# jrached/trajectory_generator_ros2

Hardware: AMD Instinct MI355X
Metric: min-snap trajectories/sec (10-seg, order-7, 3-axis) at batch=65k; 1/2/4/8 GPU (higher is better)
Workload: dtype f64

## Files before the change

include/tgms.h:

```cpp
#ifndef TGMS_H
#define TGMS_H

#include <stdint.h>

#ifdef __cplusplus
extern "C" {
#endif

#define TGMS_ABI_VERSION 2
#define TGMS_MAX_SEGMENTS 16
#define TGMS_DENSE_MAX_SEGMENTS 10
#define TGMS_GOAL_STRIDE 14

typedef enum tgms_status {
    TGMS_OK = 0,
    TGMS_ERR_INVALID_ARG = 1,
    TGMS_ERR_SINGULAR = 2,
    TGMS_ERR_NONFINITE = 3,
    TGMS_ERR_NO_DEVICE = 4,
    TGMS_ERR_DEVICE = 5,
    TGMS_ERR_UNSUPPORTED = 6,
    TGMS_ERR_SKIPPED = 7
} tgms_status;

// ... 6 lines not shown
typedef enum tgms_yaw_mode {
    TGMS_YAW_CONSTANT = 0,
    TGMS_YAW_VELOCITY = 1
} tgms_yaw_mode;

typedef struct tgms_handle tgms_handle;

int tgms_abi_version(void);
const char* tgms_status_string(int status);

tgms_status tgms_create(tgms_handle** out, int device);
tgms_status tgms_create_host(tgms_handle** out);
void tgms_destroy(tgms_handle* h);
const char* tgms_last_error(const tgms_handle* h);
tgms_status tgms_set_method(tgms_handle* h, int method);

tgms_status tgms_solve_batch(tgms_handle* h, int32_t B, const int32_t* seg_offsets,
                             const double* waypoints, const double* seg_times,
                             const double* end_derivs, double* coeffs, int32_t* status);

tgms_status tgms_solve_uniform_device(tgms_handle* h, int32_t B, int32_t M,
                                      const double* d_waypoints, const double* d_seg_times,
                                      const double* d_end_derivs, double* d_coeffs,
                                      int32_t* d_status, void* stream);
tgms_status tgms_solve_batch_device(tgms_handle* h, int32_t B, const int32_t* h_seg_offsets,
                                    const int32_t* d_seg_offsets, const double* d_waypoints,
                                    const double* d_seg_times, const double* d_end_derivs,
                                    double* d_coeffs, int32_t* d_status, void* stream);

tgms_status tgms_refine_uniform_device(tgms_handle* h, int32_t B, int32_t M, const double* d_waypoints,
// ... 8 lines not shown
                                    const int32_t* d_seg_offsets, const double* d_waypoints, double* d_seg_times,
                                    const double* d_end_derivs, double k_T, double eta, int32_t iters,
                                    double* d_coeffs, double* d_cost, int32_t* d_status, void* stream);
tgms_status tgms_refine_batch(tgms_handle* h, int32_t B, const int32_t* seg_offsets, const double* waypoints,
                              double* seg_times, const double* end_derivs, double k_T, double eta, int32_t iters,
                              double* coeffs, double* cost, int32_t* status);

int64_t tgms_sample_count(double total_T, double dt);
tgms_status tgms_sample_offsets(int32_t B, const int32_t* seg_offsets, const double* seg_times,
                                double dt, int64_t* sample_offsets);
tgms_status tgms_sample_batch(tgms_handle* h, int32_t B, const int32_t* seg_offsets,
                              const double* waypoints, const double* seg_times,
                              const double* end_derivs, const double* coeffs, double dt,
                              int yaw_mode, double yaw_const, const int64_t* sample_offsets,
                              double* out);
tgms_status tgms_sample_batch_device(tgms_handle* h, int32_t B, const int32_t* d_seg_offsets,
                                     const double* d_waypoints, const double* d_seg_times,
                                     const double* d_end_derivs, const double* d_coeffs,
                                     double dt, int yaw_mode, double yaw_const,
                                     const int64_t* d_sample_offsets, double* d_out,
                                     void* stream);

#define TGMS_EXTREMA_STRIDE 10
#define TGMS_FEAS_BOX 1
#define TGMS_FEAS_SPEED 2
#define TGMS_FEAS_ACCEL 4
#define TGMS_FEAS_JERK 8
#define TGMS_FEAS_NONFINITE 16
typedef struct tgms_limits {
    double pmin[3], pmax[3], v_max, a_max, j_max;
// ... 282 lines not shown
```

trajectory_generator_ros2_amd/_lib.py:

```python
from __future__ import annotations

import ctypes
import os

from .build import LIB_TGMS

OK, ERR_INVALID_ARG, ERR_SINGULAR, ERR_NONFINITE, ERR_NO_DEVICE, ERR_DEVICE, ERR_UNSUPPORTED, ERR_SKIPPED = range(8)
METHOD_REDUCED, METHOD_DENSE_KKT, METHOD_BAND_KKT = 0, 1, 2
YAW_CONSTANT, YAW_VELOCITY = 0, 1
ABI_VERSION = 2
MAX_SEGMENTS = 16
DENSE_MAX_SEGMENTS = 10
GOAL_STRIDE = 14
EXTREMA_STRIDE = 10
FEAS_BOX, FEAS_SPEED, FEAS_ACCEL, FEAS_JERK, FEAS_NONFINITE = 1, 2, 4, 8, 16
SEP_STRIDE = 2
SEP_CLOSE, SEP_NONFINITE = 1, 16
NEAR_NONE = -1
CLR_BAD_OBSTACLE = 32
FLD_UNRESOLVED = 64
INF_BLOCKED, INF_OUTSIDE, INF_CAPPED = 1, 2, 4
SUB_DONE, SUB_FULL, SUB_BLOCKED, SUB_OUTSIDE = 1, 2, 4, 8
SUB_MAX_DEPTH = 4
THRUST_STRIDE = 6
THRUST_LOW, THRUST_HIGH, THRUST_TILT = 1, 2, 4
RATE_STRIDE = 2
RATE_HIGH = 1
DIL_CAPPED = 1
DIL_FLAG_MASK, DIL_EVALS_SHIFT = 0xFF, 8
DIL_NONE, DIL_SPEED, DIL_ACCEL, DIL_JERK, DIL_THRUST_HIGH, DIL_THRUST_LOW, DIL_TILT = range(7)
COR_STRIDE = 2
COR_MAX_FACES = 256
COR_OUTSIDE, COR_BAD_FACE = 1, 32
SPLIT_PULL, SPLIT_CHORD = 0, 1
SPLIT_DONE, SPLIT_FULL, SPLIT_AT_END = 1, 2, 4
CUT_DONE, CUT_SNAPPED, CUT_FINISHED = 1, 2, 4

EXPORTS = [
    "tgms_abi_version", "tgms_status_string", "tgms_create", "tgms_create_host", "tgms_destroy", "tgms_last_error",
    "tgms_set_method", "tgms_solve_batch", "tgms_solve_uniform_device", "tgms_solve_batch_device",
    "tgms_sample_count", "tgms_sample_offsets", "tgms_sample_batch", "tgms_sample_batch_device",
    "tgms_refine_uniform_device", "tgms_refine_batch_device", "tgms_refine_loop_device", "tgms_refine_batch",
    "tgms_create_multi", "tgms_device_count", "tgms_plan_shards", "tgms_solve_batch_multi",
    "tgms_solve_batch_multi_device", "tgms_refine_loop_multi_device", "tgms_multi_schedule",
    "tgms_extrema_batch", "tgms_extrema_batch_device", "tgms_bounds_batch", "tgms_bounds_batch_device",
    "tgms_separation_batch", "tgms_separation_batch_device",
    "tgms_neighbors_batch", "tgms_neighbors_batch_device",
    "tgms_clearance_batch", "tgms_clearance_batch_device",
    "tgms_field_clearance_batch", "tgms_field_clearance_batch_device",
    "tgms_field_occupancy_device", "tgms_corridor_inflate_batch", "tgms_corridor_inflate_batch_device",
    "tgms_corridor_subdivide_batch", "tgms_corridor_subdivide_batch_device",
    "tgms_thrust_batch", "tgms_thrust_batch_device",
    "tgms_rate_batch", "tgms_rate_batch_device",
    "tgms_dilate_batch", "tgms_dilate_batch_device",
    "tgms_corridor_batch", "tgms_corridor_batch_device",
    "tgms_corridor_split_batch", "tgms_corridor_split_batch_device",
    "tgms_cut_batch", "tgms_cut_batch_device",
]

SCHED_REFINE, SCHED_END_DERIVS, SCHED_COEFFS, SCHED_STATUS, SCHED_COST, SCHED_SELF_GATHER = 1, 2, 4, 8, 16, 32


class Piece(ctypes.Structure):
    _fields_ = [("dev", ctypes.c_int32), ("piece", ctypes.c_int32), ("lo", ctypes.c_int32), ("hi", ctypes.c_int32),
                ("s0", ctypes.c_int64), ("s1", ctypes.c_int64), ("ws_off", ctypes.c_int64 * 11)]


class Xfer(ctypes.Structure):
    _fields_ = [("dev", ctypes.c_int32), ("piece", ctypes.c_int32), ("gather", ctypes.c_int32),
                ("array", ctypes.c_int32), ("batch_elem", ctypes.c_int64), ("ws_byte", ctypes.c_int64),
                ("count", ctypes.c_int64), ("elem_bytes", ctypes.c_int32), ("group", ctypes.c_int32)]

# ... 153 lines not shown
    L.tgms_dilate_batch.restype = ctypes.c_int
    L.tgms_corridor_batch_device.argtypes = [vp, i32, vp, vp, vp, ctypes.c_int64, vp, vp, dbl, vp, vp, vp, vp, vp, vp]
    L.tgms_corridor_batch_device.restype = ctypes.c_int
    L.tgms_corridor_batch.argtypes = [vp, i32, vp, vp, vp, ctypes.c_int64, vp, vp, dbl, vp, vp, vp, vp, vp]
    L.tgms_corridor_batch.restype = ctypes.c_int
    L.tgms_corridor_split_batch_device.argtypes = [vp, i32, vp, vp, vp, vp, ctypes.c_int64, vp, vp, vp, vp, dbl,
                                                   ctypes.c_int, dbl, vp, vp, vp, vp, vp, vp, vp, vp, vp]
    L.tgms_corridor_split_batch_device.restype = ctypes.c_int
    L.tgms_corridor_split_batch.argtypes = [vp, i32, vp, vp, vp, vp, ctypes.c_int64, vp, vp, vp, vp, dbl,
                                            ctypes.c_int, dbl, vp, vp, vp, vp, vp, vp, vp, vp]
    L.tgms_corridor_split_batch.restype = ctypes.c_int
    L.tgms_cut_batch_device.argtypes = [vp, i32, vp, vp, vp, vp, vp, vp, dbl, vp, vp, vp, vp, vp, vp, vp, vp, vp, vp]
    L.tgms_cut_batch_device.restype = ctypes.c_int
    L.tgms_cut_batch.argtypes = [vp, i32, vp, vp, vp, vp, vp, vp, dbl, vp, vp, vp, vp, vp, vp, vp, vp, vp]
    L.tgms_cut_batch.restype = ctypes.c_int
    if L.tgms_abi_version() != ABI_VERSION:
        raise ImportError(f"libtgms ABI {L.tgms_abi_version()} != {ABI_VERSION}")
    _lib = L
    return L


def status_string(status: int) -> str:
    return load().tgms_status_string(int(status)).decode()
```

trajectory_generator_ros2_amd/csrc/tgms_capi.hip:

```cpp
#include <chrono>
#include <thread>
#include <initializer_list>
#include "tgms.h"
#include "tgms_internal.h"
#include "tgms_plan.h"
#include "tgms_host.h"
#include "tgms_dilate_core.h"
#include "tgms_separation_core.h"

#include <dlfcn.h>
#include <hip/hip_runtime.h>
#include <rccl/rccl.h>

#include <algorithm>
#include <cmath>
#include <cstdio>
#include <cstdlib>
#include <cstring>
#include <functional>
#include <limits>
#include <string>
#include <vector>

#ifndef TGMS_AUX_STREAMS
#define TGMS_AUX_STREAMS 4
#endif

struct tgms_multi_ctx;

struct tgms_handle {
    bool host = false;
    int device = 0;
    tgms_multi_ctx* multi = nullptr;
    int method = TGMS_METHOD_REDUCED;
    hipStream_t stream = nullptr;
    std::string last_error;
    void* d_ws = nullptr;
    size_t ws_cap = 0;
    int32_t* d_perm = nullptr;
    size_t perm_cap = 0;
    int32_t* d_perm_hist = nullptr;
    size_t perm_hist_cap = 0;
    tgms::DevPlan* d_plan = nullptr;
    int32_t* h_perm = nullptr;
    size_t h_perm_cap = 0;
    hipEvent_t perm_ev = nullptr;
    hipEvent_t scratch_ev = nullptr;
    bool scratch_pending = false;
    double* d_loop_ws = nullptr;
    size_t loop_ws_cap = 0;
    void* d_nbr_ws = nullptr;
    size_t nbr_ws_cap = 0;
    hipStream_t aux[TGMS_AUX_STREAMS] = {};
// ... 51 lines not shown
        if (e_ != hipSuccess) return hip_err(h, e_, #call); \
    } while (0)

size_t align256(size_t x) { return (x + 255) & ~size_t(255); }

tgms_status ensure_ws(tgms_handle* h, size_t bytes) {
    if (bytes <= h->ws_cap) return TGMS_OK;
    if (h->d_ws) {
        TGMS_HIP(h, hipStreamSynchronize(h->stream));
        TGMS_HIP(h, hipFree(h->d_ws));
        h->d_ws = nullptr;
        h->ws_cap = 0;
    }
    TGMS_HIP(h, hipMalloc(&h->d_ws, bytes));
    h->ws_cap = bytes;
    return TGMS_OK;
}

tgms_status enter(tgms_handle* h, const char* gpu_only = nullptr) {
    if (!h) return TGMS_ERR_INVALID_ARG;
    if (gpu_only && h->host)
        return set_err(h, TGMS_ERR_UNSUPPORTED, std::string(gpu_only) + " needs a GPU handle (tgms_create)");
    h->last_error.clear();
    return TGMS_OK;
}

struct Region {
    void* slot;
    void (*set)(void* slot, char*);
    const void* src;
    size_t bytes;
};
template <class T>
void set_slot(void* slot, char* p) {
    *static_cast<T**>(slot) = reinterpret_cast<T*>(p);
}
template <class T>
Region input(T** dev, const T* src, size_t n) {
    return {dev, set_slot<T>, src, src ? n * sizeof(T) : 0};
}
template <class T>
Region output(T** dev, size_t n) {
    return {dev, set_slot<T>, nullptr, n * sizeof(T)};
}

tgms_status stage(tgms_handle* h, std::initializer_list<Region> regions) {
    TGMS_HIP(h, hipSetDevice(h->device));
    size_t off = 0;
    for (const Region& r : regions) off = align256(off + r.bytes);
    const tgms_status s = ensure_ws(h, off);
    if (s != TGMS_OK) return s;
    char* const base = static_cast<char*>(h->d_ws);
    off = 0;
    for (const Region& r : regions) {
        char* const d = r.bytes ? base + off : nullptr;
        r.set(r.slot, d);
        if (d && r.src) TGMS_HIP(h, hipMemcpyAsync(d, r.src, r.bytes, hipMemcpyHostToDevice, h->stream));
        off = align256(off + r.bytes);
    }
    return TGMS_OK;
}

template <class T>
hipError_t fetch(tgms_handle* h, T* host, const T* dev, size_t n) {
    return hipMemcpyAsync(host, dev, n * sizeof(T), hipMemcpyDeviceToHost, h->stream);
}

struct Outputs {
    template <class T>
    struct Part {
        size_t i;
    };
    struct Slot {
        void* host;
        size_t off, bytes;
    };
    std::vector<Slot> slots;
    size_t bytes = 0;
    char* d = nullptr;
    std::vector<char> all;

    template <class T>
    Part<T> add(T* host, size_t cap, bool reserve) {
        const size_t n = reserve ? cap * sizeof(T) : 0, off = (bytes + 15) & ~size_t(15);
        if (n) bytes = off + n;
        slots.push_back({n ? host : nullptr, off, n});
        return {slots.size() - 1};
    }
    template <class T>
    Part<T> add(T* host, size_t cap) {
        return add(host, cap, host != nullptr);
    }
    template <class T>
    T* dev(Part<T> p) const {
        return slots[p.i].bytes ? reinterpret_cast<T*>(d + slots[p.i].off) : nullptr;
    }

    tgms_status copy(tgms_handle* h, void* dst, size_t off, size_t n) const {
        TGMS_HIP(h, hipMemcpyAsync(dst, d + off, n, hipMemcpyDeviceToHost, h->stream));
        TGMS_HIP(h, hipStreamSynchronize(h->stream));
        return TGMS_OK;
    }
    tgms_status fetch(tgms_handle* h) {
        all.resize(bytes);
        return copy(h, all.data(), 0, bytes);
    }
    template <class T>
    void take(Part<T> p, size_t n) const {
        if (slots[p.i].host) std::memcpy(slots[p.i].host, all.data() + slots[p.i].off, n * sizeof(T));
    }
    tgms_status download(tgms_handle* h) {
        const Slot* only = nullptr;
        int wanted = 0;
        for (const Slot& s : slots)
            if (s.host) {
                only = &s;
                ++wanted;
            }
        if (wanted == 1) return copy(h, only->host, only->off, only->bytes);
        const tgms_status st = fetch(h);
        for (const Slot& s : slots)
            if (st == TGMS_OK && s.host) std::memcpy(s.host, all.data() + s.off, s.bytes);
        return st;
    }
};
Region output(Outputs* o) { return output(&o->d, o->bytes); }

tgms_status worst_status(tgms_handle* h, const int32_t* st, int32_t B, bool message) {
    int worst = TGMS_OK;
    for (int32_t b = 0; b < B; ++b) worst = std::max(worst, (int)st[b]);
    if (worst != TGMS_OK && message) {
        for (int32_t b = 0; b < B; ++b)
            if (st[b] == worst) {
                char buf[160];
                snprintf(buf, sizeof buf, "trajectory %d: %s", b, tgms_status_string(worst));
                h->last_error = buf;
                break;
            }
    }
    return (tgms_status)worst;
}

tgms_status finish_status(tgms_handle* h, const int32_t* dSt, int32_t* status, int32_t B, bool message) {
    std::vector<int32_t> tmp;
    if (!status) {
        tmp.resize(B);
        status = tmp.data();
    }
    TGMS_HIP(h, fetch(h, status, dSt, (size_t)B));
    TGMS_HIP(h, hipStreamSynchronize(h->stream));
    return worst_status(h, status, B, message);
}

bool capturing(hipStream_t stream) {
    hipStreamCaptureStatus cs = hipStreamCaptureStatusNone;
    return hipStreamIsCapturing(stream, &cs) == hipSuccess && cs != hipStreamCaptureStatusNone;
}

tgms_status scratch_acquire(tgms_handle* h, hipStream_t stream) {
    if (h->scratch_pending && !capturing(stream)) TGMS_HIP(h, hipStreamWaitEvent(stream, h->scratch_ev, 0));
    return TGMS_OK;
}

tgms_status scratch_release(tgms_handle* h, hipStream_t stream) {
    if (capturing(stream)) return TGMS_OK;
    TGMS_HIP(h, hipEventRecord(h->scratch_ev, stream));
// ... 1048 lines not shown
        case TGMS_ERR_DEVICE: return "TGMS_ERR_DEVICE";
        case TGMS_ERR_UNSUPPORTED: return "TGMS_ERR_UNSUPPORTED";
        case TGMS_ERR_SKIPPED: return "TGMS_ERR_SKIPPED";
        default: return "TGMS_ERR_UNKNOWN";
    }
}

tgms_status tgms_create(tgms_handle** out, int device) {
    if (!out) return TGMS_ERR_INVALID_ARG;
    *out = nullptr;
    int n = 0;
    if (hipGetDeviceCount(&n) != hipSuccess || n <= 0) return TGMS_ERR_NO_DEVICE;
    if (device < 0 || device >= n) return TGMS_ERR_INVALID_ARG;
    tgms_handle* h = new tgms_handle();
    h->device = device;
    if (hipSetDevice(device) != hipSuccess ||
        hipStreamCreateWithFlags(&h->stream, hipStreamNonBlocking) != hipSuccess ||
        hipEventCreateWithFlags(&h->perm_ev, hipEventDisableTiming) != hipSuccess ||
        hipEventCreateWithFlags(&h->scratch_ev, hipEventDisableTiming) != hipSuccess) {
        delete h;
        return TGMS_ERR_DEVICE;
    }
    *out = h;
    return TGMS_OK;
}

tgms_status tgms_create_host(tgms_handle** out) {
    if (!out) return TGMS_ERR_INVALID_ARG;
    tgms_handle* h = new tgms_handle();
    h->host = true;
// ... 3 lines not shown

void tgms_destroy(tgms_handle* h) {
    if (!h) return;
    if (h->host) {
        delete h;
        return;
    }
    if (h->multi) {
        destroy_multi(h->multi);
        h->multi = nullptr;
    }
    (void)hipSetDevice(h->device);
    if (h->stream) (void)hipStreamSynchronize(h->stream);
    (void)hipDeviceSynchronize();
    if (h->d_ws) (void)hipFree(h->d_ws);
    if (h->d_perm_hist) (void)hipFree(h->d_perm_hist);
    if (h->d_band) (void)hipFree(h->d_band);
    if (h->d_band_graph) (void)hipFree(h->d_band_graph);
    for (double* p : h->band_retired) (void)hipFree(p);
    if (h->d_perm) (void)hipFree(h->d_perm);
    if (h->h_perm) (void)hipHostFree(h->h_perm);
    if (h->perm_ev) (void)hipEventDestroy(h->perm_ev);
    if (h->scratch_ev) (void)hipEventDestroy(h->scratch_ev);
    if (h->band_done) (void)hipHostFree(h->band_done);
    if (h->d_loop_ws) (void)hipFree(h->d_loop_ws);
    if (h->d_nbr_ws) (void)hipFree(h->d_nbr_ws);
    for (int j = 0; j < TGMS_AUX_STREAMS; ++j) {
        if (h->aux[j]) (void)hipStreamDestroy(h->aux[j]);
        if (h->join_ev[j]) (void)hipEventDestroy(h->join_ev[j]);
    }
    if (h->fork_ev) (void)hipEventDestroy(h->fork_ev);
    for (auto& g : h->loop_graphs) {
        if (g.done) (void)hipEventSynchronize(g.done);
        if (g.exec) (void)hipGraphExecDestroy(g.exec);
        if (g.done) (void)hipEventDestroy(g.done);
    }
    if (h->d_plan) (void)hipFree(h->d_plan);
    if (h->cap_stream) (void)hipStreamDestroy(h->cap_stream);
    if (h->stream) (void)hipStreamDestroy(h->stream);
    (void)hipGetLastError();
    delete h;
}

const char* tgms_last_error(const tgms_handle* h) { return h ? h->last_error.c_str() : ""; }

tgms_status tgms_set_method(tgms_handle* h, int method) {
    if (!h) return TGMS_ERR_INVALID_ARG;
    if (method != TGMS_METHOD_REDUCED && method != TGMS_METHOD_DENSE_KKT && method != TGMS_METHOD_BAND_KKT)
        return set_err(h, TGMS_ERR_INVALID_ARG, "unknown method");
    if (h->host && method != TGMS_METHOD_REDUCED)
        return set_err(h, TGMS_ERR_UNSUPPORTED, "the host backend solves the reduced formulation only");
    h->method = method;
    if (h->multi)
        for (tgms_handle* sub : h->multi->sub)
            if (sub) sub->method = method;
    return TGMS_OK;
}

tgms_status tgms_solve_batch(tgms_handle* h, int32_t B, const int32_t* so, const double* waypoints,
                             const double* seg_times, const double* end_derivs, double* coeffs,
// ... 8 lines not shown
    if (h->host) {
        int worst = TGMS_OK;
        for (int32_t b = 0; b < B; ++b) {
            const int64_t s0 = so[b];
            const int st = tgms::host::solve(so[b + 1] - so[b], waypoints + (s0 + b) * 3, seg_times + s0,
                                             end_derivs ? end_derivs + (int64_t)b * 18 : nullptr, coeffs + s0 * 24);
            if (status) status[b] = st;
            if (st > worst) {
                worst = st;
                h->last_error = "trajectory " + std::to_string(b) + ": " + tgms_status_string(st);
            }
        }
        return (tgms_status)worst;
    }
    const size_t S = (size_t)so[B];
    double *dW, *dT, *dED, *dC;
    int32_t *dSt, *dSo;
    s = stage(h, {input(&dW, waypoints, (S + B) * 3), input(&dT, seg_times, S), input(&dED, end_derivs, (size_t)B * 18),
                  output(&dC, S * 24), output(&dSt, (size_t)B), input(&dSo, so, (size_t)B + 1)});
    if (s != TGMS_OK) return s;
    hipStream_t st = h->stream;
    s = scratch_acquire(h, st);
    if (s != TGMS_OK) return s;
    s = plan_upload(h, B, so, &plan, st);
    if (s != TGMS_OK) return s;
    s = scratch_release(h, st, dispatch(h, plan, B, dSo, dW, dT, dED, dC, dSt, st));
    if (s != TGMS_OK) return s;
    TGMS_HIP(h, fetch(h, coeffs, dC, S * 24));
    return finish_status(h, dSt, status, B, true);
}

static bool misaligned(std::initializer_list<const void*> ps) {
    for (const void* p : ps)
        if (p && (reinterpret_cast<uintptr_t>(p) & 15u)) return true;
    return false;
}
#define TGMS_CHECK_ALIGNED(h, ...)                                                                   \
    do {                                                                                             \
        if (misaligned({__VA_ARGS__}))                                                               \
            return set_err(h, TGMS_ERR_INVALID_ARG, "fp64 device buffers must be 16-byte aligned"); \
    } while (0)

tgms_status tgms_solve_uniform_device(tgms_handle* h, int32_t B, int32_t M, const double* dW,
                                      const double* dT, const double* dED, double* dC,
// ... 82 lines not shown
}

tgms_status tgms_refine_batch(tgms_handle* h, int32_t B, const int32_t* so, const double* waypoints,
                              double* seg_times, const double* end_derivs, double k_T, double eta, int32_t iters,
                              double* coeffs, double* cost, int32_t* status) {
    if (tgms_status e = enter(h, __func__); e != TGMS_OK) return e;
    tgms_status s = check_refine_args(h, k_T, eta);
    if (s != TGMS_OK) return s;
    if (iters < 0) return set_err(h, TGMS_ERR_INVALID_ARG, "iters < 0");
    Plan plan;
    s = scan_offsets(h, B, so, TGMS_MAX_SEGMENTS, &plan.uniform_m);
    if (s != TGMS_OK) return s;
    if (B == 0) return TGMS_OK;
    if (!waypoints || !seg_times) return set_err(h, TGMS_ERR_INVALID_ARG, "NULL waypoints/seg_times");
    const size_t S = (size_t)so[B];
    double *dW, *dT[2], *dED, *dC, *dCost;
    int32_t *dSt, *dSo;
    s = stage(h, {input(&dW, waypoints, (S + B) * 3), input(&dT[0], seg_times, S), output(&dT[1], S),
                  input(&dED, end_derivs, (size_t)B * 18), output(&dC, coeffs ? S * 24 : 0), output(&dCost, (size_t)B),
                  output(&dSt, (size_t)B), input(&dSo, so, (size_t)B + 1)});
    if (s != TGMS_OK) return s;
    hipStream_t st = h->stream;
    s = scratch_acquire(h, st);
    if (s == TGMS_OK && plan.uniform_m == 0) s = ensure_perm_device(h, B);
    if (s != TGMS_OK) return s;
    const DevPlanBufs dp{h->d_perm_hist, h->d_perm, h->d_plan};
    int cur = 0;
    s = scratch_release(h, st, refine_loop(h, plan, B, (int64_t)S, dSo, dW, dT, dED, k_T, eta, iters, dC, dCost, dSt,
                                           st, &cur, &dp));
    if (s != TGMS_OK) return s;
    if (coeffs) TGMS_HIP(h, fetch(h, coeffs, dC, S * 24));
    TGMS_HIP(h, fetch(h, seg_times, dT[cur], S));
    if (cost) TGMS_HIP(h, fetch(h, cost, dCost, (size_t)B));
    return finish_status(h, dSt, status, B, false);
}

tgms_status tgms_refine_loop_device(tgms_handle* h, int32_t B, const int32_t* h_so, const int32_t* d_so,
                                    const double* dW, double* dT, const double* dED, double k_T, double eta,
                                    int32_t iters, double* dC, double* d_cost, int32_t* dSt, void* stream) {
    if (tgms_status e = enter(h, __func__); e != TGMS_OK) return e;
    tgms_status s = check_refine_args(h, k_T, eta);
    if (s != TGMS_OK) return s;
    if (iters < 0) return set_err(h, TGMS_ERR_INVALID_ARG, "iters < 0");
    int um = 0;
    s = scan_offsets(h, B, h_so, TGMS_MAX_SEGMENTS, &um);
    if (s != TGMS_OK) return s;
    if (B == 0) return TGMS_OK;
    if (!d_so || !dW || !dT) return set_err(h, TGMS_ERR_INVALID_ARG, "NULL device pointer");
    TGMS_CHECK_ALIGNED(h, dW, dT, dED, dC, d_cost);
    hipStream_t st = static_cast<hipStream_t>(stream);
    s = no_capture(h, st, "tgms_refine_loop_device (it captures and replays its own graph)");
    if (s == TGMS_OK) s = scratch_acquire(h, st);
    if (s != TGMS_OK) return s;
    return scratch_release(h, st, loop_on_device(h, B, (int64_t)h_so[B], um, d_so, dW, dT, dED, k_T, eta, iters, dC,
                                                 d_cost, dSt, st));
}

int64_t tgms_sample_count(double total_T, double dt) {
    if (!(dt > 0.0) || !(total_T >= 0.0) || !std::isfinite(total_T)) return 0;
    const double x = std::ceil(total_T / dt - 1e-9);
    int64_t n = (int64_t)x;
    if (n < 1) n = 1;
    return n + 1;
}

tgms_status tgms_sample_offsets(int32_t B, const int32_t* so, const double* T, double dt,
                                int64_t* sample_offsets) {
    if (B < 0 || !so || !sample_offsets || (B > 0 && !T) || !(dt > 0.0)) return TGMS_ERR_INVALID_ARG;
    sample_offsets[0] = 0;
    for (int32_t b = 0; b < B; ++b) {
// ... 32 lines not shown
    if (B == 0) return TGMS_OK;
    if (!waypoints || !seg_times || !coeffs || !sample_offsets || !out || !(dt > 0.0))
        return set_err(h, TGMS_ERR_INVALID_ARG, "NULL pointer or dt <= 0");
    if (yaw_mode != TGMS_YAW_CONSTANT && yaw_mode != TGMS_YAW_VELOCITY)
        return set_err(h, TGMS_ERR_INVALID_ARG, "bad yaw_mode");
    if (h->host) {
        for (int32_t b = 0; b < B; ++b) {
            const int64_t s0 = so[b];
            tgms::host::sample(so[b + 1] - so[b], coeffs + s0 * 24, seg_times + s0, waypoints + (s0 + b) * 3,
                               end_derivs ? end_derivs + (int64_t)b * 18 : nullptr, dt, yaw_mode, yaw_const,
                               sample_offsets[b + 1] - sample_offsets[b], out + sample_offsets[b] * TGMS_GOAL_STRIDE);
        }
        return TGMS_OK;
    }
    const size_t S = (size_t)so[B], nOut = (size_t)sample_offsets[B] * TGMS_GOAL_STRIDE;
    double *dW, *dT, *dED, *dC, *dOut;
    int32_t* dSo;
    int64_t* dSmp;
    s = stage(h, {input(&dW, waypoints, (S + B) * 3), input(&dT, seg_times, S), input(&dED, end_derivs, (size_t)B * 18),
                  input(&dC, coeffs, S * 24), input(&dSo, so, (size_t)B + 1),
                  input(&dSmp, sample_offsets, (size_t)B + 1), output(&dOut, nOut)});
    if (s != TGMS_OK) return s;
    TGMS_HIP(h, tgms::launch_sample(B, dSo, dW, dT, dED, dC, dt, yaw_mode, yaw_const, dSmp, dOut, h->stream));
    TGMS_HIP(h, fetch(h, out, dOut, nOut));
    TGMS_HIP(h, hipStreamSynchronize(h->stream));
    return TGMS_OK;
}


static bool resolve_limits(const tgms_limits* in, tgms_limits* out) {
    const double inf = std::numeric_limits<double>::infinity();
    if (!in) {
        *out = tgms_limits{{-inf, -inf, -inf}, {inf, inf, inf}, inf, inf, inf};
        return true;
    }
    *out = *in;
    for (int a = 0; a < 3; ++a)
        if (!(in->pmin[a] <= in->pmax[a])) return false;
    return !(std::isnan(in->v_max) || std::isnan(in->a_max) || std::isnan(in->j_max));
}

// ... 1190 lines not shown
    a.iters = iters;
    return multi_run(h, a, static_cast<hipStream_t>(stream));
}

tgms_status tgms_solve_batch_multi(tgms_handle* h, int32_t B, const int32_t* so, const double* waypoints,
                                   const double* seg_times, const double* end_derivs, double* coeffs,
                                   int32_t* status) {
    if (tgms_status e = enter(h, __func__); e != TGMS_OK) return e;
    if (!h->multi) return tgms_solve_batch(h, B, so, waypoints, seg_times, end_derivs, coeffs, status);
    Plan checked;
    tgms_status s = check_offsets(h, B, so, max_m_for(h), &checked.counts, &checked.uniform_m);
    if (s != TGMS_OK || B == 0) return s;
    if (!waypoints || !seg_times || !coeffs)
        return set_err(h, TGMS_ERR_INVALID_ARG, "NULL waypoints/seg_times/coeffs");
    const size_t S = (size_t)so[B];
    double *dW, *dT, *dED, *dC;
    int32_t *dSt, *dSo;
    s = stage(h, {input(&dW, waypoints, (S + B) * 3), input(&dT, seg_times, S), input(&dED, end_derivs, (size_t)B * 18),
                  output(&dC, S * 24), output(&dSt, (size_t)B), input(&dSo, so, (size_t)B + 1)});
    if (s != TGMS_OK) return s;
    MultiArgs a;
    a.checked = &checked;
    a.B = B;
    a.h_so = so;
    a.d_so = dSo;
    a.dW = dW;
    a.dT = dT;
    a.dED = dED;
    a.dC = dC;
    a.dSt = dSt;
    s = multi_run(h, a, h->stream);
    (void)hipSetDevice(h->device);
    if (s != TGMS_OK) return s;
    TGMS_HIP(h, fetch(h, coeffs, dC, S * 24));
    return finish_status(h, dSt, status, B, true);
}

}
```

trajectory_generator_ros2_amd/host/MinSnap.cpp:

```cpp
#include "MinSnap.hpp"

#include <algorithm>
#include <cmath>
#include <cstdlib>
#include <string>

namespace trajectory_generator {

namespace {

GoalMsg to_goal(const double* s) {
    GoalMsg g;
    g.header.frame_id = "world";
    g.p.x = s[0];
    g.p.y = s[1];
    g.p.z = s[2];
    g.v.x = s[3];
    g.v.y = s[4];
    g.v.z = s[5];
    g.a.x = s[6];
    g.a.y = s[7];
    g.a.z = s[8];
    g.j.x = s[9];
    g.j.y = s[10];
// ... 32 lines not shown
    }
    return h_;
}

bool MinSnap::solve_and_sample(const std::vector<double>& W, const std::vector<double>& T, const double* end_derivs,
                               std::vector<double>& coeffs, std::vector<double>& samples, std::string& err) {
    tgms_handle* h = handle();
    if (!h) {
        err = p_.host_backend ? "no host solver" : "no GPU solver";
        return false;
    }
    const int32_t M = (int32_t)T.size();
    const int32_t so[2] = {0, M};
    int32_t st = TGMS_OK;
    coeffs.assign((size_t)M * 24, 0.0);
    tgms_status s = tgms_solve_batch(h, 1, so, W.data(), T.data(), end_derivs, coeffs.data(), &st);
    if (s != TGMS_OK || st != TGMS_OK) {
        err = std::string("solve failed: ") + tgms_status_string(s != TGMS_OK ? s : st) + " " + tgms_last_error(h);
        return false;
    }
    int64_t offs[2];
    s = tgms_sample_offsets(1, so, T.data(), dt_, offs);
    if (s != TGMS_OK) {
        err = std::string("sample_offsets failed: ") + tgms_status_string(s);
        return false;
    }
    samples.assign((size_t)offs[1] * TGMS_GOAL_STRIDE, 0.0);
    s = tgms_sample_batch(h, 1, so, W.data(), T.data(), end_derivs, coeffs.data(), dt_, p_.yaw_mode, p_.yaw, offs,
                          samples.data());
    if (s != TGMS_OK) {
        err = std::string("sampling failed: ") + tgms_status_string(s) + " " + tgms_last_error(h);
        return false;
    }
    return true;
}

bool MinSnap::ensure_main() {
    if (solved_) return true;
    std::string err;
    if (!solve_and_sample(p_.waypoints, p_.seg_times, nullptr, coeffs_, samples_, err)) {
        log_error("MinSnap traj: %s", err.c_str());
        return false;
    }
    solved_ = true;
    return true;
}
// ... 105 lines not shown
```

trajectory_generator_ros2_amd/solver.py:

```python
from __future__ import annotations

import ctypes
from typing import Optional, Tuple

import numpy as np

from . import _lib
from ._lib import TgmsError


def _ptr(a) -> Optional[int]:
    if a is None:
        return None
    if isinstance(a, np.ndarray):
        assert a.flags.c_contiguous, "arrays must be C-contiguous"
        return a.ctypes.data
    assert a.is_contiguous(), "tensors must be contiguous"
    return a.data_ptr()


class Solver:

    def __init__(self, device: int = 0, method: int = _lib.METHOD_REDUCED, device_count: int = 0,
                 host: bool = False):
# ... 79 lines not shown
    def sample(self, seg_offsets, waypoints, seg_times, end_derivs, coeffs, dt: float,
               yaw_mode: int = _lib.YAW_CONSTANT, yaw_const: float = 0.0):
        so = np.ascontiguousarray(seg_offsets, dtype=np.int32)
        W = np.ascontiguousarray(waypoints, dtype=np.float64).reshape(-1, 3)
        T = np.ascontiguousarray(seg_times, dtype=np.float64).reshape(-1)
        ED = None if end_derivs is None else np.ascontiguousarray(end_derivs, dtype=np.float64).reshape(-1, 18)
        C = np.ascontiguousarray(coeffs, dtype=np.float64)
        B = so.shape[0] - 1
        offs = sample_offsets(so, T, dt)
        out = np.zeros((int(offs[-1]), _lib.GOAL_STRIDE), dtype=np.float64)
        st = self._L.tgms_sample_batch(self._h, B, _ptr(so), _ptr(W), _ptr(T), _ptr(ED), _ptr(C), float(dt),
                                       int(yaw_mode), float(yaw_const), _ptr(offs), _ptr(out))
        if st != _lib.OK:
            raise TgmsError(st, self.last_error())
        return offs, out

    def extrema(self, seg_offsets, waypoints, seg_times, end_derivs, coeffs, dt: float,
                limits: Optional[_lib.Limits] = None) -> Tuple[np.ndarray, np.ndarray]:
        so = np.ascontiguousarray(seg_offsets, dtype=np.int32)
        W = np.ascontiguousarray(waypoints, dtype=np.float64).reshape(-1, 3)
        T = np.ascontiguousarray(seg_times, dtype=np.float64).reshape(-1)
        ED = None if end_derivs is None else np.ascontiguousarray(end_derivs, dtype=np.float64).reshape(-1, 18)
        C = np.ascontiguousarray(coeffs, dtype=np.float64)
        B = so.shape[0] - 1
        ext = np.zeros((B, _lib.EXTREMA_STRIDE), dtype=np.float64)
        flags = np.zeros(B, dtype=np.int32)
        st = self._L.tgms_extrema_batch(self._h, B, _ptr(so), _ptr(W), _ptr(T), _ptr(ED), _ptr(C), float(dt),
                                        None if limits is None else ctypes.byref(limits), _ptr(ext), _ptr(flags))
        if st != _lib.OK:
            raise TgmsError(st, self.last_error())
# ... 577 lines not shown
```

Before: 2.313 billion.

## Stage small host transfers through pinned mirror buffer and add fused solve+sample

Adds a pinned host mirror of the device workspace. Below a size threshold, inputs are packed into it and uploaded with one contiguous copy, and outputs are read back with one contiguous copy into the mirror. A new solve+sample entry point runs both stages on one stage/upload. It also replaces the separate per-output fetches and syncs with grouped asynchronous downloads. The aim is to cut per-call copy and sync overhead for small batches, at the cost of extra host memcpy and a pinned allocation.

```diff
diff --git a/include/tgms.h b/include/tgms.h
--- a/include/tgms.h
+++ b/include/tgms.h
@@ -44,6 +44,10 @@
 void tgms_destroy(tgms_handle* h);
 const char* tgms_last_error(const tgms_handle* h);
 tgms_status tgms_set_method(tgms_handle* h, int method);
+
+#define TGMS_STAGE_THRESHOLD_DEFAULT 131072
+int64_t tgms_stage_threshold(const tgms_handle* h);
+int64_t tgms_alloc_count(const tgms_handle* h);
 
 tgms_status tgms_solve_batch(tgms_handle* h, int32_t B, const int32_t* seg_offsets,
                              const double* waypoints, const double* seg_times,
@@ -82,6 +86,11 @@
                               const double* end_derivs, const double* coeffs, double dt,
                               int yaw_mode, double yaw_const, const int64_t* sample_offsets,
                               double* out);
+tgms_status tgms_solve_sample_batch(tgms_handle* h, int32_t B, const int32_t* seg_offsets,
+                                    const double* waypoints, const double* seg_times,
+                                    const double* end_derivs, double dt, int yaw_mode, double yaw_const,
+                                    const int64_t* sample_offsets, double* coeffs, int32_t* status,
+                                    double* out);
 tgms_status tgms_sample_batch_device(tgms_handle* h, int32_t B, const int32_t* d_seg_offsets,
                                      const double* d_waypoints, const double* d_seg_times,
                                      const double* d_end_derivs, const double* d_coeffs,
diff --git a/trajectory_generator_ros2_amd/_lib.py b/trajectory_generator_ros2_amd/_lib.py
--- a/trajectory_generator_ros2_amd/_lib.py
+++ b/trajectory_generator_ros2_amd/_lib.py
@@ -35,6 +35,7 @@
 SPLIT_PULL, SPLIT_CHORD = 0, 1
 SPLIT_DONE, SPLIT_FULL, SPLIT_AT_END = 1, 2, 4
 CUT_DONE, CUT_SNAPPED, CUT_FINISHED = 1, 2, 4
+STAGE_THRESHOLD_DEFAULT = 131072
 
 EXPORTS = [
     "tgms_abi_version", "tgms_status_string", "tgms_create", "tgms_create_host", "tgms_destroy", "tgms_last_error",
@@ -56,6 +57,7 @@
     "tgms_corridor_batch", "tgms_corridor_batch_device",
     "tgms_corridor_split_batch", "tgms_corridor_split_batch_device",
     "tgms_cut_batch", "tgms_cut_batch_device",
+    "tgms_solve_sample_batch", "tgms_stage_threshold", "tgms_alloc_count",
 ]
 
 SCHED_REFINE, SCHED_END_DERIVS, SCHED_COEFFS, SCHED_STATUS, SCHED_COST, SCHED_SELF_GATHER = 1, 2, 4, 8, 16, 32
@@ -239,6 +241,12 @@
     L.tgms_cut_batch_device.restype = ctypes.c_int
     L.tgms_cut_batch.argtypes = [vp, i32, vp, vp, vp, vp, vp, vp, dbl, vp, vp, vp, vp, vp, vp, vp, vp, vp]
     L.tgms_cut_batch.restype = ctypes.c_int
+    L.tgms_solve_sample_batch.argtypes = [vp, i32, vp, vp, vp, vp, dbl, ctypes.c_int, dbl, vp, vp, vp, vp]
+    L.tgms_solve_sample_batch.restype = ctypes.c_int
+    L.tgms_stage_threshold.argtypes = [vp]
+    L.tgms_stage_threshold.restype = i64
+    L.tgms_alloc_count.argtypes = [vp]
+    L.tgms_alloc_count.restype = i64
     if L.tgms_abi_version() != ABI_VERSION:
         raise ImportError(f"libtgms ABI {L.tgms_abi_version()} != {ABI_VERSION}")
     _lib = L
diff --git a/trajectory_generator_ros2_amd/csrc/tgms_capi.hip b/trajectory_generator_ros2_amd/csrc/tgms_capi.hip
--- a/trajectory_generator_ros2_amd/csrc/tgms_capi.hip
+++ b/trajectory_generator_ros2_amd/csrc/tgms_capi.hip
@@ -4,6 +4,7 @@
 #include "tgms.h"
 #include "tgms_internal.h"
 #include "tgms_plan.h"
+#include "tgms_stage_plan.h"
 #include "tgms_host.h"
 #include "tgms_dilate_core.h"
 #include "tgms_separation_core.h"
@@ -37,6 +38,12 @@
     std::string last_error;
     void* d_ws = nullptr;
     size_t ws_cap = 0;
+    char* h_pin = nullptr;
+    size_t pin_cap = 0;
+    size_t stage_threshold = TGMS_STAGE_THRESHOLD_DEFAULT;
+    size_t mirror = 0;
+    bool pin_inflight = false;
+    int64_t ws_allocs = 0;
     int32_t* d_perm = nullptr;
     size_t perm_cap = 0;
     int32_t* d_perm_hist = nullptr;
@@ -118,6 +125,27 @@
     }
     TGMS_HIP(h, hipMalloc(&h->d_ws, bytes));
     h->ws_cap = bytes;
+    ++h->ws_allocs;
+    return TGMS_OK;
+}
+
+tgms_status ensure_pin(tgms_handle* h, size_t bytes) {
+    if (bytes <= h->pin_cap) return TGMS_OK;
+    if (h->h_pin) {
+        TGMS_HIP(h, hipStreamSynchronize(h->stream));
+        TGMS_HIP(h, hipHostFree(h->h_pin));
+        h->h_pin = nullptr;
+        h->pin_cap = 0;
+    }
+    TGMS_HIP(h, hipHostMalloc(reinterpret_cast<void**>(&h->h_pin), bytes));
+    h->pin_cap = bytes;
+    ++h->ws_allocs;
+    return TGMS_OK;
+}
+
+tgms_status drain(tgms_handle* h) {
+    TGMS_HIP(h, hipStreamSynchronize(h->stream));
+    h->pin_inflight = false;
     return TGMS_OK;
 }
 
@@ -148,21 +176,56 @@
     return {dev, set_slot<T>, nullptr, n * sizeof(T)};
 }
 
+constexpr size_t STAGE_MAX_REGIONS = 16;
+
 tgms_status stage(tgms_handle* h, std::initializer_list<Region> regions) {
     TGMS_HIP(h, hipSetDevice(h->device));
-    size_t off = 0;
-    for (const Region& r : regions) off = align256(off + r.bytes);
-    const tgms_status s = ensure_ws(h, off);
+    tgms::StageRegion sr[STAGE_MAX_REGIONS];
+    size_t off[STAGE_MAX_REGIONS], n = 0;
+    if (regions.size() > STAGE_MAX_REGIONS) return set_err(h, TGMS_ERR_INVALID_ARG, "stage: too many regions");
+    for (const Region& r : regions) sr[n++] = {r.bytes, r.src != nullptr};
+    const tgms::StagePlan plan = tgms::stage_plan(sr, n, h->stage_threshold, off);
+    h->mirror = 0;
+    if (h->pin_inflight) {
+        const tgms_status s = drain(h);
+        if (s != TGMS_OK) return s;
+    }
+    tgms_status s = ensure_ws(h, plan.total);
+    if (s == TGMS_OK && plan.staged) s = ensure_pin(h, plan.mirror);
     if (s != TGMS_OK) return s;
     char* const base = static_cast<char*>(h->d_ws);
-    off = 0;
+    size_t i = 0;
     for (const Region& r : regions) {
-        char* const d = r.bytes ? base + off : nullptr;
+        char* const d = r.bytes ? base + off[i] : nullptr;
         r.set(r.slot, d);
-        if (d && r.src) TGMS_HIP(h, hipMemcpyAsync(d, r.src, r.bytes, hipMemcpyHostToDevice, h->stream));
-        off = align256(off + r.bytes);
-    }
-    return TGMS_OK;
+        if (d && r.src) {
+            if (plan.staged)
+                std::memcpy(h->h_pin + off[i], r.src, r.bytes);
+            else
+                TGMS_HIP(h, hipMemcpyAsync(d, r.src, r.bytes, hipMemcpyHostToDevice, h->stream));
+        }
+        ++i;
+    }
+    if (plan.staged) {
+        h->pin_inflight = true;
+        h->mirror = plan.mirror;
+        TGMS_HIP(h, hipMemcpyAsync(base + plan.lo, h->h_pin + plan.lo, plan.hi - plan.lo, hipMemcpyHostToDevice,
+                                   h->stream));
+    }
+    return TGMS_OK;
+}
+
+bool mirrored(const tgms_handle* h, const void* dev_end) {
+    const char* const base = static_cast<const char*>(h->d_ws);
+    return h->mirror && dev_end > h->d_ws && (size_t)(static_cast<const char*>(dev_end) - base) <= h->mirror;
+}
+char* mirror_of(const tgms_handle* h, const void* dev) {
+    return h->h_pin + (static_cast<const char*>(dev) - static_cast<const char*>(h->d_ws));
+}
+tgms_status fetch_mirror(tgms_handle* h, const void* lo, const void* hi) {
+    const size_t n = static_cast<const char*>(hi) - static_cast<const char*>(lo);
+    if (n) TGMS_HIP(h, hipMemcpyAsync(mirror_of(h, lo), lo, n, hipMemcpyDeviceToHost, h->stream));
+    return drain(h);
 }
 
 template <class T>
@@ -183,6 +246,7 @@
     size_t bytes = 0;
     char* d = nullptr;
     std::vector<char> all;
+    const char* got = nullptr;
 
     template <class T>
     Part<T> add(T* host, size_t cap, bool reserve) {
@@ -200,18 +264,32 @@
         return slots[p.i].bytes ? reinterpret_cast<T*>(d + slots[p.i].off) : nullptr;
     }
 
+    bool small(const tgms_handle* h) const { return mirrored(h, d + bytes); }
     tgms_status copy(tgms_handle* h, void* dst, size_t off, size_t n) const {
+        if (small(h)) {
+            const tgms_status st = fetch_mirror(h, d + off, d + off + n);
+            if (st == TGMS_OK) std::memcpy(dst, mirror_of(h, d + off), n);
+            return st;
+        }
         TGMS_HIP(h, hipMemcpyAsync(dst, d + off, n, hipMemcpyDeviceToHost, h->stream));
-        TGMS_HIP(h, hipStreamSynchronize(h->stream));
-        return TGMS_OK;
-    }
-    tgms_status fetch(tgms_handle* h) {
+        return drain(h);
+    }
+    tgms_status fetch(tgms_handle* h, size_t from = 0) {
+        if (small(h)) {
+            got = mirror_of(h, d);
+            return fetch_mirror(h, d + from, d + bytes);
+        }
         all.resize(bytes);
-        return copy(h, all.data(), 0, bytes);
+        got = all.data();
+        return copy(h, all.data() + from, from, bytes - from);
     }
     template <class T>
     void take(Part<T> p, size_t n) const {
-        if (slots[p.i].host) std::memcpy(slots[p.i].host, all.data() + slots[p.i].off, n * sizeof(T));
+        if (slots[p.i].host) std::memcpy(slots[p.i].host, got + slots[p.i].off, n * sizeof(T));
+    }
+    template <class T>
+    const T* view(Part<T> p) const {
+        return reinterpret_cast<const T*>(got + slots[p.i].off);
     }
     tgms_status download(tgms_handle* h) {
         const Slot* only = nullptr;
@@ -224,7 +302,7 @@
         if (wanted == 1) return copy(h, only->host, only->off, only->bytes);
         const tgms_status st = fetch(h);
         for (const Slot& s : slots)
-            if (st == TGMS_OK && s.host) std::memcpy(s.host, all.data() + s.off, s.bytes);
+            if (st == TGMS_OK && s.host) std::memcpy(s.host, got + s.off, s.bytes);
         return st;
     }
 };
@@ -252,8 +330,25 @@
         status = tmp.data();
     }
     TGMS_HIP(h, fetch(h, status, dSt, (size_t)B));
-    TGMS_HIP(h, hipStreamSynchronize(h->stream));
-    return worst_status(h, status, B, message);
+    const tgms_status s = drain(h);
+    return s != TGMS_OK ? s : worst_status(h, status, B, message);
+}
+
+tgms_status finish_solve(tgms_handle* h, Outputs& out, Outputs::Part<int32_t> oSt, size_t from, int32_t B,
+                         bool message) {
+    if (out.small(h)) {
+        const tgms_status s = out.fetch(h, from);
+        if (s != TGMS_OK) return s;
+        for (const Outputs::Slot& sl : out.slots)
+            if (sl.host) std::memcpy(sl.host, out.got + sl.off, sl.bytes);
+        return worst_status(h, out.view(oSt), B, message);
+    }
+    for (size_t i = 0; i < out.slots.size(); ++i) {
+        const Outputs::Slot& sl = out.slots[i];
+        if (sl.host && i != oSt.i)
+            TGMS_HIP(h, hipMemcpyAsync(sl.host, out.d + sl.off, sl.bytes, hipMemcpyDeviceToHost, h->stream));
+    }
+    return finish_status(h, out.dev(oSt), static_cast<int32_t*>(out.slots[oSt.i].host), B, message);
 }
 
 bool capturing(hipStream_t stream) {
@@ -1332,6 +1427,11 @@
     if (device < 0 || device >= n) return TGMS_ERR_INVALID_ARG;
     tgms_handle* h = new tgms_handle();
     h->device = device;
+    if (const char* t = std::getenv("TGMS_STAGE_THRESHOLD")) {
+        char* end = nullptr;
+        const unsigned long long v = std::strtoull(t, &end, 10);
+        h->stage_threshold = end != t ? (size_t)v : std::string(t) == "inf" ? ~size_t(0) : h->stage_threshold;
+    }
     if (hipSetDevice(device) != hipSuccess ||
         hipStreamCreateWithFlags(&h->stream, hipStreamNonBlocking) != hipSuccess ||
         hipEventCreateWithFlags(&h->perm_ev, hipEventDisableTiming) != hipSuccess ||
@@ -1365,6 +1465,7 @@
     if (h->stream) (void)hipStreamSynchronize(h->stream);
     (void)hipDeviceSynchronize();
     if (h->d_ws) (void)hipFree(h->d_ws);
+    if (h->h_pin) (void)hipHostFree(h->h_pin);
     if (h->d_perm_hist) (void)hipFree(h->d_perm_hist);
     if (h->d_band) (void)hipFree(h->d_band);
     if (h->d_band_graph) (void)hipFree(h->d_band_graph);
@@ -1395,6 +1496,13 @@
 
 const char* tgms_last_error(const tgms_handle* h) { return h ? h->last_error.c_str() : ""; }
 
+int64_t tgms_stage_threshold(const tgms_handle* h) {
+    if (!h || h->host) return 0;
+    return h->stage_threshold > (size_t)INT64_MAX ? INT64_MAX : (int64_t)h->stage_threshold;
+}
+
+int64_t tgms_alloc_count(const tgms_handle* h) { return h ? h->ws_allocs : 0; }
+
 tgms_status tgms_set_method(tgms_handle* h, int method) {
     if (!h) return TGMS_ERR_INVALID_ARG;
     if (method != TGMS_METHOD_REDUCED && method != TGMS_METHOD_DENSE_KKT && method != TGMS_METHOD_BAND_KKT)
@@ -1433,20 +1541,22 @@
         return (tgms_status)worst;
     }
     const size_t S = (size_t)so[B];
-    double *dW, *dT, *dED, *dC;
-    int32_t *dSt, *dSo;
+    double *dW, *dT, *dED;
+    int32_t* dSo;
+    Outputs out;
+    const auto oC = out.add(coeffs, S * 24);
+    const auto oSt = out.add(status, (size_t)B, true);
     s = stage(h, {input(&dW, waypoints, (S + B) * 3), input(&dT, seg_times, S), input(&dED, end_derivs, (size_t)B * 18),
-                  output(&dC, S * 24), output(&dSt, (size_t)B), input(&dSo, so, (size_t)B + 1)});
+                  input(&dSo, so, (size_t)B + 1), output(&out)});
     if (s != TGMS_OK) return s;
     hipStream_t st = h->stream;
     s = scratch_acquire(h, st);
     if (s != TGMS_OK) return s;
     s = plan_upload(h, B, so, &plan, st);
     if (s != TGMS_OK) return s;
-    s = scratch_release(h, st, dispatch(h, plan, B, dSo, dW, dT, dED, dC, dSt, st));
-    if (s != TGMS_OK) return s;
-    TGMS_HIP(h, fetch(h, coeffs, dC, S * 24));
-    return finish_status(h, dSt, status, B, true);
+    s = scratch_release(h, st, dispatch(h, plan, B, dSo, dW, dT, dED, out.dev(oC), out.dev(oSt), st));
+    if (s != TGMS_OK) return s;
+    return finish_solve(h, out, oSt, 0, B, true);
 }
 
 static bool misaligned(std::initializer_list<const void*> ps) {
@@ -1559,12 +1669,17 @@
     if (B == 0) return TGMS_OK;
     if (!waypoints || !seg_times) return set_err(h, TGMS_ERR_INVALID_ARG, "NULL waypoints/seg_times");
     const size_t S = (size_t)so[B];
-    double *dW, *dT[2], *dED, *dC, *dCost;
-    int32_t *dSt, *dSo;
-    s = stage(h, {input(&dW, waypoints, (S + B) * 3), input(&dT[0], seg_times, S), output(&dT[1], S),
-                  input(&dED, end_derivs, (size_t)B * 18), output(&dC, coeffs ? S * 24 : 0), output(&dCost, (size_t)B),
-                  output(&dSt, (size_t)B), input(&dSo, so, (size_t)B + 1)});
-    if (s != TGMS_OK) return s;
+    double *dW, *dT[2], *dED;
+    int32_t* dSo;
+    Outputs out;
+    const auto oC = out.add(coeffs, S * 24);
+    const auto oCost = out.add(cost, (size_t)B, true);
+    const auto oSt = out.add(status, (size_t)B, true);
+    s = stage(h, {input(&dW, waypoints, (S + B) * 3), input(&dED, end_derivs, (size_t)B * 18),
+                  input(&dSo, so, (size_t)B + 1), input(&dT[0], seg_times, S), output(&dT[1], S), output(&out)});
+    if (s != TGMS_OK) return s;
+    double *const dC = out.dev(oC), *const dCost = out.dev(oCost);
+    int32_t* const dSt = out.dev(oSt);
     hipStream_t st = h->stream;
     s = scratch_acquire(h, st);
     if (s == TGMS_OK && plan.uniform_m == 0) s = ensure_perm_device(h, B);
@@ -1574,10 +1689,18 @@
     s = scratch_release(h, st, refine_loop(h, plan, B, (int64_t)S, dSo, dW, dT, dED, k_T, eta, iters, dC, dCost, dSt,
                                            st, &cur, &dp));
     if (s != TGMS_OK) return s;
-    if (coeffs) TGMS_HIP(h, fetch(h, coeffs, dC, S * 24));
+    if (out.small(h)) {
+        out.got = mirror_of(h, out.d);
+        s = fetch_mirror(h, dT[cur], out.d + out.bytes);
+        if (s != TGMS_OK) return s;
+        std::memcpy(seg_times, mirror_of(h, dT[cur]), S * sizeof(double));
+        out.take(oC, S * 24);
+        out.take(oCost, (size_t)B);
+        out.take(oSt, (size_t)B);
+        return worst_status(h, out.view(oSt), B, false);
+    }
     TGMS_HIP(h, fetch(h, seg_times, dT[cur], S));
-    if (cost) TGMS_HIP(h, fetch(h, cost, dCost, (size_t)B));
-    return finish_status(h, dSt, status, B, false);
+    return finish_solve(h, out, oSt, 0, B, false);
 }
 
 tgms_status tgms_refine_loop_device(tgms_handle* h, int32_t B, const int32_t* h_so, const int32_t* d_so,
@@ -1599,6 +1722,51 @@
     if (s != TGMS_OK) return s;
     return scratch_release(h, st, loop_on_device(h, B, (int64_t)h_so[B], um, d_so, dW, dT, dED, k_T, eta, iters, dC,
                                                  d_cost, dSt, st));
+}
+
+tgms_status tgms_solve_sample_batch(tgms_handle* h, int32_t B, const int32_t* so, const double* waypoints,
+                                    const double* seg_times, const double* end_derivs, double dt, int yaw_mode,
+                                    double yaw_const, const int64_t* sample_offsets, double* coeffs, int32_t* status,
+                                    double* out) {
+    if (tgms_status e = enter(h); e != TGMS_OK) return e;
+    Plan plan;
+    tgms_status s = check_offsets(h, B, so, max_m_for(h), &plan.counts, &plan.uniform_m);
+    if (s != TGMS_OK) return s;
+    if (B == 0) return TGMS_OK;
+    if (!waypoints || !seg_times || !sample_offsets || !out || !(dt > 0.0))
+        return set_err(h, TGMS_ERR_INVALID_ARG, "NULL pointer or dt <= 0");
+    if (yaw_mode != TGMS_YAW_CONSTANT && yaw_mode != TGMS_YAW_VELOCITY)
+        return set_err(h, TGMS_ERR_INVALID_ARG, "bad yaw_mode");
+    const size_t S = (size_t)so[B], nOut = (size_t)sample_offsets[B] * TGMS_GOAL_STRIDE;
+    if (h->host) {
+        std::vector<double> tmp(coeffs ? 0 : S * 24);
+        double* const C = coeffs ? coeffs : tmp.data();
+        const tgms_status worst = tgms_solve_batch(h, B, so, waypoints, seg_times, end_derivs, C, status);
+        const std::string msg = h->last_error;
+        s = tgms_sample_batch(h, B, so, waypoints, seg_times, end_derivs, C, dt, yaw_mode, yaw_const, sample_offsets, out);
+        if (s != TGMS_OK) return s;
+        h->last_error = msg;
+        return worst;
+    }
+    double *dW, *dT, *dED;
+    int32_t* dSo;
+    int64_t* dSmp;
+    Outputs o;
+    const auto oC = o.add(coeffs, S * 24, true);
+    const auto oSt = o.add(status, (size_t)B, true);
+    const auto oOut = o.add(out, nOut);
+    s = stage(h, {input(&dW, waypoints, (S + B) * 3), input(&dT, seg_times, S), input(&dED, end_derivs, (size_t)B * 18),
+                  input(&dSo, so, (size_t)B + 1), input(&dSmp, sample_offsets, (size_t)B + 1), output(&o)});
+    if (s != TGMS_OK) return s;
+    hipStream_t st = h->stream;
+    s = scratch_acquire(h, st);
+    if (s != TGMS_OK) return s;
+    s = plan_upload(h, B, so, &plan, st);
+    if (s != TGMS_OK) return s;
+    s = scratch_release(h, st, dispatch(h, plan, B, dSo, dW, dT, dED, o.dev(oC), o.dev(oSt), st));
+    if (s != TGMS_OK) return s;
+    TGMS_HIP(h, tgms::launch_sample(B, dSo, dW, dT, dED, o.dev(oC), dt, yaw_mode, yaw_const, dSmp, o.dev(oOut), st));
+    return finish_solve(h, o, oSt, coeffs ? 0 : o.slots[oSt.i].off, B, true);
 }
 
 int64_t tgms_sample_count(double total_T, double dt) {
@@ -1661,17 +1829,17 @@
         return TGMS_OK;
     }
     const size_t S = (size_t)so[B], nOut = (size_t)sample_offsets[B] * TGMS_GOAL_STRIDE;
-    double *dW, *dT, *dED, *dC, *dOut;
+    double *dW, *dT, *dED, *dC;
     int32_t* dSo;
     int64_t* dSmp;
+    Outputs o;
+    const auto oOut = o.add(out, nOut);
     s = stage(h, {input(&dW, waypoints, (S + B) * 3), input(&dT, seg_times, S), input(&dED, end_derivs, (size_t)B * 18),
                   input(&dC, coeffs, S * 24), input(&dSo, so, (size_t)B + 1),
-                  input(&dSmp, sample_offsets, (size_t)B + 1), output(&dOut, nOut)});
-    if (s != TGMS_OK) return s;
-    TGMS_HIP(h, tgms::launch_sample(B, dSo, dW, dT, dED, dC, dt, yaw_mode, yaw_const, dSmp, dOut, h->stream));
-    TGMS_HIP(h, fetch(h, out, dOut, nOut));
-    TGMS_HIP(h, hipStreamSynchronize(h->stream));
-    return TGMS_OK;
+                  input(&dSmp, sample_offsets, (size_t)B + 1), output(&o)});
+    if (s != TGMS_OK) return s;
+    TGMS_HIP(h, tgms::launch_sample(B, dSo, dW, dT, dED, dC, dt, yaw_mode, yaw_const, dSmp, o.dev(oOut), h->stream));
+    return o.download(h);
 }
 
 
@@ -2892,10 +3060,13 @@
     if (!waypoints || !seg_times || !coeffs)
         return set_err(h, TGMS_ERR_INVALID_ARG, "NULL waypoints/seg_times/coeffs");
     const size_t S = (size_t)so[B];
-    double *dW, *dT, *dED, *dC;
-    int32_t *dSt, *dSo;
+    double *dW, *dT, *dED;
+    int32_t* dSo;
+    Outputs out;
+    const auto oC = out.add(coeffs, S * 24);
+    const auto oSt = out.add(status, (size_t)B, true);
     s = stage(h, {input(&dW, waypoints, (S + B) * 3), input(&dT, seg_times, S), input(&dED, end_derivs, (size_t)B * 18),
-                  output(&dC, S * 24), output(&dSt, (size_t)B), input(&dSo, so, (size_t)B + 1)});
+                  input(&dSo, so, (size_t)B + 1), output(&out)});
     if (s != TGMS_OK) return s;
     MultiArgs a;
     a.checked = &checked;
@@ -2905,13 +3076,12 @@
     a.dW = dW;
     a.dT = dT;
     a.dED = dED;
-    a.dC = dC;
-    a.dSt = dSt;
+    a.dC = out.dev(oC);
+    a.dSt = out.dev(oSt);
     s = multi_run(h, a, h->stream);
     (void)hipSetDevice(h->device);
     if (s != TGMS_OK) return s;
-    TGMS_HIP(h, fetch(h, coeffs, dC, S * 24));
-    return finish_status(h, dSt, status, B, true);
-}
-
-}
+    return finish_solve(h, out, oSt, 0, B, true);
+}
+
+}
diff --git a/trajectory_generator_ros2_amd/csrc/tgms_stage_plan.h b/trajectory_generator_ros2_amd/csrc/tgms_stage_plan.h
--- /dev/null
+++ b/trajectory_generator_ros2_amd/csrc/tgms_stage_plan.h
@@ -0,0 +1,47 @@
+#pragma once
+
+#include <cstddef>
+
+namespace tgms {
+
+constexpr size_t STAGE_MIRROR_FACTOR = 8;
+
+struct StageRegion {
+    size_t bytes;
+    bool input;
+};
+
+struct StagePlan {
+    size_t total = 0;
+    size_t in_bytes = 0;
+    size_t lo = 0, hi = 0;
+    bool staged = false;
+    size_t mirror = 0;
+};
+
+inline size_t stage_align(size_t x) { return (x + 255) & ~size_t(255); }
+
+inline StagePlan stage_plan(const StageRegion* r, size_t n, size_t threshold, size_t* off) {
+    StagePlan p;
+    size_t o = 0;
+    bool any = false;
+    for (size_t i = 0; i < n; ++i) {
+        off[i] = o;
+        if (r[i].input && r[i].bytes) {
+            if (!any) p.lo = o;
+            any = true;
+            p.hi = o + r[i].bytes;
+            p.in_bytes += r[i].bytes;
+        }
+        o = stage_align(o + r[i].bytes);
+    }
+    p.total = o;
+    p.staged = any && p.in_bytes <= threshold;
+    if (p.staged) {
+        const size_t cap = threshold > ~size_t(0) / STAGE_MIRROR_FACTOR ? ~size_t(0) : threshold * STAGE_MIRROR_FACTOR;
+        p.mirror = p.total <= cap ? p.total : p.hi;
+    }
+    return p;
+}
+
+}
diff --git a/trajectory_generator_ros2_amd/host/MinSnap.cpp b/trajectory_generator_ros2_amd/host/MinSnap.cpp
--- a/trajectory_generator_ros2_amd/host/MinSnap.cpp
+++ b/trajectory_generator_ros2_amd/host/MinSnap.cpp
@@ -70,22 +70,21 @@
     const int32_t so[2] = {0, M};
     int32_t st = TGMS_OK;
     coeffs.assign((size_t)M * 24, 0.0);
-    tgms_status s = tgms_solve_batch(h, 1, so, W.data(), T.data(), end_derivs, coeffs.data(), &st);
+    int64_t offs[2];
+    tgms_status s = tgms_sample_offsets(1, so, T.data(), dt_, offs);
+    if (s != TGMS_OK) {
+        s = tgms_solve_batch(h, 1, so, W.data(), T.data(), end_derivs, coeffs.data(), &st);
+        if (s != TGMS_OK || st != TGMS_OK)
+            err = std::string("solve failed: ") + tgms_status_string(s != TGMS_OK ? s : st) + " " + tgms_last_error(h);
+        else
+            err = std::string("sample_offsets failed: ") + tgms_status_string(TGMS_ERR_INVALID_ARG);
+        return false;
+    }
+    samples.assign((size_t)offs[1] * TGMS_GOAL_STRIDE, 0.0);
+    s = tgms_solve_sample_batch(h, 1, so, W.data(), T.data(), end_derivs, dt_, p_.yaw_mode, p_.yaw, offs, coeffs.data(),
+                                &st, samples.data());
     if (s != TGMS_OK || st != TGMS_OK) {
         err = std::string("solve failed: ") + tgms_status_string(s != TGMS_OK ? s : st) + " " + tgms_last_error(h);
-        return false;
-    }
-    int64_t offs[2];
-    s = tgms_sample_offsets(1, so, T.data(), dt_, offs);
-    if (s != TGMS_OK) {
-        err = std::string("sample_offsets failed: ") + tgms_status_string(s);
-        return false;
-    }
-    samples.assign((size_t)offs[1] * TGMS_GOAL_STRIDE, 0.0);
-    s = tgms_sample_batch(h, 1, so, W.data(), T.data(), end_derivs, coeffs.data(), dt_, p_.yaw_mode, p_.yaw, offs,
-                          samples.data());
-    if (s != TGMS_OK) {
-        err = std::string("sampling failed: ") + tgms_status_string(s) + " " + tgms_last_error(h);
         return false;
     }
     return true;
diff --git a/trajectory_generator_ros2_amd/solver.py b/trajectory_generator_ros2_amd/solver.py
--- a/trajectory_generator_ros2_amd/solver.py
+++ b/trajectory_generator_ros2_amd/solver.py
@@ -117,6 +117,31 @@
         if st != _lib.OK:
             raise TgmsError(st, self.last_error())
         return offs, out
+
+    def solve_sample(self, seg_offsets, waypoints, seg_times, end_derivs, dt: float,
+                     yaw_mode: int = _lib.YAW_CONSTANT, yaw_const: float = 0.0, want_coeffs: bool = True):
+        so = np.ascontiguousarray(seg_offsets, dtype=np.int32)
+        W = np.ascontiguousarray(waypoints, dtype=np.float64).reshape(-1, 3)
+        T = np.ascontiguousarray(seg_times, dtype=np.float64).reshape(-1)
+        ED = None if end_derivs is None else np.ascontiguousarray(end_derivs, dtype=np.float64).reshape(-1, 18)
+        B = so.shape[0] - 1
+        S = int(so[-1]) if B > 0 else 0
+        offs = sample_offsets(so, T, dt)
+        C = np.zeros((S, 3, 8), dtype=np.float64) if want_coeffs else None
+        st = np.zeros(max(B, 1), dtype=np.int32)
+        out = np.zeros((int(offs[-1]), _lib.GOAL_STRIDE), dtype=np.float64)
+        worst = self._L.tgms_solve_sample_batch(self._h, B, _ptr(so), _ptr(W), _ptr(T), _ptr(ED), float(dt),
+                                                int(yaw_mode), float(yaw_const), _ptr(offs), _ptr(C), _ptr(st),
+                                                _ptr(out))
+        if worst in (_lib.ERR_DEVICE, _lib.ERR_NO_DEVICE):
+            raise TgmsError(worst, self.last_error())
+        return C, st[:B], worst, offs, out
+
+    def stage_threshold(self) -> int:
+        return int(self._L.tgms_stage_threshold(self._h))
+
+    def alloc_count(self) -> int:
+        return int(self._L.tgms_alloc_count(self._h))
 
     def extrema(self, seg_offsets, waypoints, seg_times, end_derivs, coeffs, dt: float,
                 limits: Optional[_lib.Limits] = None) -> Tuple[np.ndarray, np.ndarray]:
```

Result: slower. 2.269 billion (-1.9%).
